# CESNET/GPUJPEG

Measured on AMD Instinct MI355X. Metric: Mpix/s encode+decode (8K RGB q75), higher is better.
Workload: dtype f32

## Files before the change

gpujpeg_amd/csrc/gj_dec_entropy_tok.hip:

```cpp
#include "gj_dec_internal.h"
#include "gj_bitreader.h"

#ifndef GJ_TOK_SUB
#define GJ_TOK_SUB 16
#define GJ_TOK_SUB_MAX 20
#endif
#define GJ_TOK_MAX_SUBS (GJ_TOK_CAP_U / GJ_TOK_SUB + (GJ_TOK_SUB <= 17 ? GJ_TOK_GMAX / 2 : GJ_TOK_GMAX))
#define GJ_TOK_WSTAGE 944
#define GJ_TOK_WG_PER_CU 4
#ifndef GJ_TOK_SYNC
#define GJ_TOK_SYNC 48
#endif
#define GJ_TOK_CHUNK_MAX 48

#ifdef GJ_TRACE_PHASES
static __device__ unsigned long long* gj_trace_buf;
extern "C" GJ_HIP_API int gj_hip_trace_set(void* p) { return hipMemcpyToSymbol(HIP_SYMBOL(gj_trace_buf), &p, sizeof p) == hipSuccess ? 0 : -1; }
#define GJ_TRACE(slot) do { if (threadIdx.x == 0 && gj_trace_buf) gj_trace_buf[(size_t)blockIdx.x * 16 + (slot)] = __builtin_amdgcn_s_memrealtime(); } while (0)
#else
#define GJ_TRACE(slot) ((void)0)
#endif

#ifdef GJ_TOK_STATS
extern "C" GJ_HIP_API unsigned long long gj_tok_stats[64];
unsigned long long gj_tok_stats[64];
#define GJ_STAT_WAVE(sm, i, lane, sym) do { gj_wave_sync(); (sm).statsym[threadIdx.x] = (sym); gj_wave_sync(); if ((lane) == 0) { \
    unsigned long long s_ = 0, m_ = 0; for (int q_ = 0; q_ < 64; q_++) { const unsigned v_ = (sm).statsym[(threadIdx.x & ~63) + q_]; s_ += v_; if (v_ > m_) m_ = v_; } \
    GJ_STAT(i, s_); GJ_STAT((i) + 1, 64 * m_); GJ_STAT((i) + 2, 1); } } while (0)
#define GJ_SYMS(c) (((c) >> 16) + 2u * ((c) & 0xFFFFu))
#define GJ_STAT(i, n) __atomic_fetch_add(&gj_tok_stats[i], (unsigned long long)(n), __ATOMIC_RELAXED)
#else
#define GJ_STAT(i, n) ((void)0)
#define GJ_STAT_WAVE(sm, i, lane, sym) ((void)0)
#endif

#ifndef GJ_TOK_WIN
#define GJ_TOK_WIN 1
#endif
#if GJ_TOK_WIN == 1
#define GJ_TOK_WIN_INIT(sm, p1) uint32_t wcur_ = (p1) >> 5, w0_ = (sm).U[wcur_], w1_ = (sm).U[wcur_ + 1], wnx_ = 0
#define GJ_TOK_WIN_BITS(sm, p1) wnx_ = (sm).U[wcur_ + 2]; const uint32_t win = __builtin_amdgcn_alignbit(w0_, w1_, ~(p1))
#define GJ_TOK_WIN_STEP(p1) do { const uint32_t wn_ = (p1) >> 5; const bool cross_ = wn_ != wcur_; w0_ = cross_ ? w1_ : w0_; w1_ = cross_ ? wnx_ : w1_; wcur_ = wn_; } while (0)
#else
#define GJ_TOK_WIN_INIT(sm, p1) ((void)0)
#define GJ_TOK_WIN_BITS(sm, p1) const uint32_t wi = (p1) >> 5; const uint32_t win = __builtin_amdgcn_alignbit((sm).U[wi], (sm).U[wi + 1], ~(p1))
#define GJ_TOK_WIN_STEP(p1) ((void)0)
#endif


struct GjTokLds {
    uint32_t U[GJ_TOK_CAP_U / 4 + 8];
    __attribute__((aligned(16))) uint16_t tab[2 * GJ_DEC2_WORDS];
    __attribute__((aligned(8))) uint2 rec[GJ_TOK_MAX_SUBS];
    __attribute__((aligned(16))) uint16_t pool[(GJ_TOK_MAX_BLOCKS + GJ_TOK_GMAX) * 2 + 4 * GJ_TOK_WSTAGE];
    uint32_t bb[GJ_TOK_GMAX + 1], cap[GJ_TOK_GMAX + 1], first[GJ_TOK_GMAX];
    uint16_t tabsel[GJ_TOK_GMAX];
    uint32_t sbit[GJ_TOK_GMAX], ebit[GJ_TOK_GMAX], sub0[GJ_TOK_GMAX + 1];
    uint32_t tmp[4];
    uint32_t nwork[2], big;
    uint32_t gpos;
    uint8_t zz[64 + 64];
#ifdef GJ_TOK_STATS
    uint32_t statsym[256];
#endif
};

__device__ __forceinline__ uint32_t gj_tok_run_in(const GjTokLds& sm, const uint32_t from, const uint32_t start_bit)
{
    uint32_t p1 = from - 1u;
    const uint32_t e1 = start_bit - 1u;
    uint32_t z = 1;
    uint32_t toff = (uint32_t)GJ_DEC2_WORDS * 2u;
    GJ_TOK_WIN_INIT(sm, p1);
    while (p1 < e1) {
        GJ_TOK_WIN_BITS(sm, p1);
        const uint16_t* t = reinterpret_cast<const uint16_t*>(reinterpret_cast<const uint8_t*>(sm.tab) + toff);
        uint32_t e = t[gj_bfe_u32<32 - GJ_DEC_FAST_BITS, GJ_DEC_FAST_BITS>(win)];
        if ((e & 31u) == 0) e = t[(e >> 5) + ((win >> 16) & 63u)];
        p1 += e & 31u;
        GJ_TOK_WIN_STEP(p1);
        z += (e >> 9) & 63u;
        const uint32_t inside = (uint32_t)((int32_t)(z - 64u) >> 31);
        z &= inside;
        toff = ((uint32_t)GJ_DEC2_WORDS * 2u) & inside;
    }
    return (p1 - e1) | (z << 5);
}

template <int MODE>
__device__ __forceinline__ uint32_t gj_tok_decode(const GjTokLds& sm, const uint32_t start_bit, const uint32_t end_bit, const uint32_t entry, uint32_t& counts,
                                                  uint16_t* __restrict__ tok_out ,
                                                  uint32_t* __restrict__ s_blkinfo ,
                                                  const uint32_t tok_rel , uint32_t blk,
                                                  const uint32_t nblocks, int16_t* __restrict__ coefs ,
                                                  uint32_t* __restrict__ s_big)
{
    uint32_t p1 = start_bit + (entry & 31u) - 1u;
    const uint32_t e1 = end_bit - 1u;
    uint32_t z = (entry >> 5) & 63u;
    uint32_t toff = z == 0 ? 0u : (uint32_t)GJ_DEC2_WORDS * 2u;
    uint32_t nb = 0, ntok = 0, mx = 0;
    uint16_t* tp = tok_out;
    GJ_TOK_WIN_INIT(sm, p1);
    while (p1 < e1) {
        GJ_TOK_WIN_BITS(sm, p1);
        const uint16_t* t = reinterpret_cast<const uint16_t*>(reinterpret_cast<const uint8_t*>(sm.tab) + toff);
        uint32_t e = t[gj_bfe_u32<32 - GJ_DEC_FAST_BITS, GJ_DEC_FAST_BITS>(win)];
        if ((e & 31u) == 0) e = t[(e >> 5) + ((win >> 16) & 63u)];
        const uint32_t tot = e & 31u, adv = (e >> 9) & 63u, sz = (e >> 5) & 15u;
        if (MODE == 0) {
            ntok += e >> 15;
        } else {
            const uint32_t x = win << (tot - sz);
            uint32_t neg = (uint32_t)((int32_t)~x >> 31);
            GJ_KEEP(neg);
            const uint32_t mag = (x ^ neg) >> ((32u - sz) & 31u);
            const int v = (int)((mag ^ neg) - neg);
            if ((int16_t)e < 0) {
                const uint32_t pos = z + adv - 1u;
                if (MODE == 1) {
                    mx = max(mx, sz);
                    *tp++ = (uint16_t)(((uint32_t)v << 6) | sm.zz[pos]);
                } else {
                    if (blk + nb < nblocks && pos < 64u) coefs[(uint64_t)(blk + nb) * 64 + sm.zz[pos]] = (int16_t)v;
                    ntok++;
                }
            } else if (z == 0) {
                const uint32_t t = MODE == 1 ? tok_rel + (uint32_t)(tp - tok_out) : tok_rel + ntok;
                if (blk + nb <= nblocks) s_blkinfo[blk + nb] = (sz ? (uint32_t)v & 0xFFFFu : 0u) | (t << 16);
            }
        }
        p1 += tot;
        GJ_TOK_WIN_STEP(p1);
        z += adv;
        const uint32_t inside = (uint32_t)((int32_t)(z - 64u) >> 31);
        z &= inside;
        toff = ((uint32_t)GJ_DEC2_WORDS * 2u) & inside;
        nb += 1u + inside;
    }
    if (MODE == 1) ntok = (uint32_t)(tp - tok_out);
    if (MODE == 1 && mx >= 10u) *s_big = 1u;
    counts = nb | (ntok << 16);
    return (p1 - e1) | (z << 5);
}

template <bool COOP>
__global__ __launch_bounds__(256, GJ_TOK_WG_PER_CU) void k_huffman_decode_tok(const gj_geom g, const uint8_t* __restrict__ jpeg, uint64_t jpeg_size,
                                                               const uint32_t* __restrict__ seg_pos, const uint32_t* __restrict__ seg_len,
                                                               const uint32_t* __restrict__ seg_index, const int seg_count_max,
                                                               const uint32_t* __restrict__ seg_count_ptr, const GjBatchPlan plan,
                                                               const uint16_t* __restrict__ tabs, int16_t* __restrict__ coefs,
                                                               uint16_t* __restrict__ d_tok, const uint32_t tok_cap, uint2* __restrict__ d_rec,
                                                               uint32_t* __restrict__ overflow, const GjFold F)
{
    constexpr int CAP_U = GJ_TOK_CAP_U, MAX_BLOCKS = GJ_TOK_MAX_BLOCKS, GMAX = GJ_TOK_GMAX, MAX_SUBS = GJ_TOK_MAX_SUBS;
    if (g.fb.sizes != nullptr) {
        const size_t z = blockIdx.z;
        jpeg += z * g.fb.jpeg;
        jpeg_size = g.fb.sizes[z];
        seg_pos += z * g.fb.seg; seg_len += z * g.fb.seg; seg_index += z * g.fb.seg;
        if (seg_count_ptr) seg_count_ptr += z * (sizeof(gj_scan_summary) / 4);
        overflow += z * (sizeof(gj_scan_summary) / 4);
        coefs += z * g.fb.coefs; d_tok += z * g.fb.tok; d_rec += z * g.fb.rec;
    }
    __shared__ GjTokLds sm;
    constexpr int POOL = sizeof(sm.pool) / 2;
    uint32_t* const s_stage = sm.U + 1;
    uint16_t* const s_pool = sm.pool;
    uint32_t* const s_blkinfo = reinterpret_cast<uint32_t*>(sm.pool);
    uint2* const s_rec = sm.rec;
    uint32_t *const s_bb = sm.bb, *const s_cap = sm.cap, *const s_first = sm.first, *const s_sbit = sm.sbit, *const s_ebit = sm.ebit, *const s_sub0 = sm.sub0;
    uint32_t* const s_tmp = sm.tmp;
    constexpr int BORROW = ((4 * GMAX + 1) * 2 + 7) & ~7;
    uint32_t* const s_pos = reinterpret_cast<uint32_t*>(s_pool + POOL - BORROW);
    uint32_t* const s_len = s_pos + GMAX;
    uint32_t* const s_ubyte = s_len + GMAX;
    uint32_t* const s_ulen = s_ubyte + GMAX + 1;
    static_assert(BORROW <= GJ_TOK_WSTAGE && MAX_SUBS <= POOL - BORROW, "borrowed space");
    uint16_t* const s_work = s_pool;

    const int tid = threadIdx.x, lane = tid & 63, wave = tid >> 6;
    GJ_TRACE(0);
    uint32_t sel_of_lane = 0x0C0C0C0Cu;
    {
        int at = 3;
#pragma unroll
        for (int k = 0; k < 4; k++)
            if (lane & (1 << k)) { sel_of_lane = (sel_of_lane & ~(0xFFu << (8 * at))) | ((uint32_t)k << (8 * at)); at--; }
    }
    if (tid < 128) sm.zz[tid] = tid < 64 ? GJ_ZZ[tid] : 0;
    if (tid == 0) sm.U[0] = 0;
    const uint32_t* end = reinterpret_cast<const uint32_t*>((reinterpret_cast<uintptr_t>(jpeg) + jpeg_size + 3) & ~(uintptr_t)3);

    int pc = 0;
    while (pc + 1 < plan.n && (int)blockIdx.x >= plan.batch0[pc + 1]) pc++;
    const int G = plan.g[pc];
    const int si0 = plan.first[pc] + ((int)blockIdx.x - plan.batch0[pc]) * G;
    uint32_t ld_s = 0xFFFFFFFFu, ld_p = 0, ld_l = 0;
    if (F.recs == nullptr && tid < G && si0 + tid < seg_count_max) { ld_s = seg_index[si0 + tid]; ld_p = seg_pos[si0 + tid]; ld_l = seg_len[si0 + tid]; }
    const int seg_count = seg_count_ptr ? min((int)*seg_count_ptr, seg_count_max) : seg_count_max;
    if (si0 >= seg_count) return;
    const int nseg = min(min(G, plan.first[pc] + plan.count[pc] - si0), seg_count - si0);
    if (F.recs != nullptr) {
        static_assert(GJ_FOLD_SCRATCH_WORDS(GJ_TOK_GMAX) * 2 <= (GJ_TOK_MAX_BLOCKS + GJ_TOK_GMAX) * 2, "fold scratch inside the block slots");
        if (!gj_fold_batch<GJ_TOK_GMAX>(F, g, jpeg, jpeg_size, plan, pc, si0, nseg, reinterpret_cast<uint32_t*>(sm.pool), s_tmp, ld_s, ld_p, ld_l)) return;
    }
    uint32_t loaded_tabs = 0xFFFFFFFFu;
    auto load_tables = [&](const uint32_t tb) {
        const uint4* src0 = reinterpret_cast<const uint4*>(tabs + (tb & 0xFFu) * GJ_DEC2_WORDS);
        const uint4* src1 = reinterpret_cast<const uint4*>(tabs + (tb >> 8) * GJ_DEC2_WORDS);
        uint4* dst = reinterpret_cast<uint4*>(sm.tab);
        for (int t = tid; t < GJ_DEC2_WORDS / 8; t += 256) { dst[t] = src0[t]; dst[GJ_DEC2_WORDS / 8 + t] = src1[t]; }
        loaded_tabs = tb;
    };
    if (plan.n > 1 && plan.n == g.comp_count) load_tables((uint32_t)(g.comp[pc].dc_table * 2 + 0) | ((uint32_t)(g.comp[pc].ac_table * 2 + 1) << 8));
    uint32_t my_pos = 0, my_len = 0, my_nblk = 0;
    {
        uint32_t first = 0, tb = 0;
        if (tid < nseg) {
            const uint32_t s = ld_s, p_ = ld_p, l_ = ld_l;
            if (s < (uint32_t)g.segment_count) {
                const GjSeg sg = gj_segment(g, (int)s);
                const gj_comp_geom& kc = g.comp[sg.comp];
                my_nblk = (uint32_t)sg.nblocks;
                my_pos = p_;
                my_len = l_;
                first = (uint32_t)(kc.data_offset / 64) + (uint32_t)sg.mcu_first;
                tb = (uint32_t)(kc.dc_table * 2 + 0) | ((uint32_t)(kc.ac_table * 2 + 1) << 8);
                if (((my_len + 3u) & ~3u) + 8u > (uint32_t)CAP_U || my_nblk > (uint32_t)MAX_BLOCKS) {
                    *overflow = 1u;
                    my_len = 0;
                    my_nblk = 0;
                }
            }
        }
        if (tid < GMAX) {
            s_first[tid] = first;
            sm.tabsel[tid] = (uint16_t)tb;
        }
        if (wave == 0) {
            s_bb[tid + 1] = gj_wave_incl_scan(tid < nseg ? my_nblk + 1u : 0u);
            s_cap[tid + 1] = gj_wave_incl_scan(my_len ? ((my_len + 3u) & ~3u) + 8u : 0u);
        }
        if (tid == 0) { s_bb[0] = 0; s_cap[0] = 0; sm.nwork[0] = 0; sm.nwork[1] = 0; }
    }
    static_assert(GMAX == 64, "one wave holds the batch's segment table");
    __syncthreads();
    const uint32_t stage0 = (2u * s_bb[nseg] + 7u) & ~7u, stage_cap = (((uint32_t)POOL - stage0) >> 2) & ~7u;
    uint16_t* const stage = s_pool + stage0 + (uint32_t)wave * stage_cap;

    for (int j0 = 0; j0 < nseg;) {
        if (tid == 0) sm.big = 0;
        if (tid < nseg) { s_pos[tid] = my_pos; s_len[tid] = my_len; }
        {
            const unsigned long long mb = __ballot(lane >= j0 && lane < nseg && my_nblk != 0u);
            if (wave == 0 && lane == (mb ? (int)__builtin_ctzll(mb) : j0)) sm.gpos = my_pos;
        }
        const uint32_t tb = sm.tabsel[j0];
        const bool other = lane > j0 && lane < nseg && s_bb[lane + 1] - s_bb[lane] != 1u && sm.tabsel[lane] != tb;
        const unsigned long long mo = __ballot(other);
        const int jstop = mo ? (int)__builtin_ctzll(mo) : nseg;
        const unsigned long long mf = __ballot(lane + 1 > j0 && lane + 1 <= jstop && s_cap[lane + 1] - s_cap[j0] <= (uint32_t)CAP_U);
        const int j1 = max(j0 + 1, mf ? 64 - (int)__builtin_clzll(mf) : 0);
        const int ng = j1 - j0;
        if (COOP) {
            const uint32_t n16 = min((s_cap[j1] - s_cap[j0] + 16u + 4u + 15u) >> 4, (uint32_t)(sizeof(sm.U) / 16));
            uint4* const z = reinterpret_cast<uint4*>(sm.U);
            for (uint32_t t = (uint32_t)tid; t < n16; t += 256u) z[t] = uint4{0u, 0u, 0u, 0u};
        }
        __syncthreads();
        GJ_TRACE(1);

        if (tb != loaded_tabs) load_tables(tb);

        bool coop = false;
        if (COOP) {
            bool irregular = false;
            if (lane < ng) {
                const int j = j0 + lane;
                irregular = s_len[j] == 0 || (lane + 1 < ng && s_pos[j + 1] != s_pos[j] + s_len[j] + 2u);
            }
            const uint32_t A = s_pos[j0], total = s_pos[j1 - 1] + s_len[j1 - 1] - A;
            coop = __ballot(irregular) == 0ull && total <= 256u * GJ_TOK_CHUNK_MAX && A >= 8u && (uint64_t)A + total <= jpeg_size;
        }
        if (coop) {
            const uint32_t A = s_pos[j0], total = s_pos[j1 - 1] + s_len[j1 - 1] - A;
            const uint32_t C = (((total + 255u) >> 8) + 3u) & ~3u;
            const uint32_t off0 = (uint32_t)tid * C;
            const uintptr_t a = reinterpret_cast<uintptr_t>(jpeg) + A + off0;
            const uint32_t* src = reinterpret_cast<const uint32_t*>(a & ~(uintptr_t)3) - 1;
            const uint32_t lead = (uint32_t)((reinterpret_cast<uintptr_t>(jpeg) + A) & 3);
            uint32_t win[GJ_TOK_CHUNK_MAX / 4 + 3];
#pragma unroll
            for (int i = 0; i < GJ_TOK_CHUNK_MAX / 4 + 3; i++) {
                win[i] = 0;
                if ((uint32_t)i < C / 4 + 3u && off0 < total + 4u && src + i < end) win[i] = src[i];
            }
            constexpr int ND = GJ_TOK_CHUNK_MAX / 4;
            uint64_t keep = 0, mark = 0;
            {
                const uint32_t K7 = 0x7F7F7F7Fu, K8 = 0x80808080u;
                uint32_t eq_prev = 0, m2_prev = 0, st_prev = 0;
                uint32_t ffc = 0;
                if (off0 != 0) {
                    const uint32_t x = __builtin_amdgcn_alignbyte(win[1], win[0], lead);
                    ffc = ((x & K7) + 0x01010101u) & x & K8;
                }
#pragma unroll
                for (int i = 0; i <= ND; i++) {
                    if ((uint32_t)(4 * i) <= C) {
                        const uint32_t x = __builtin_amdgcn_alignbyte(win[i + 2], win[i + 1], lead);
                        const uint32_t t = x & K7;
                        const uint32_t eq = (t + 0x01010101u) & x & K8;
                        const uint32_t zr = ~((t + K7) | x) & K8;
                        const uint32_t y = (x ^ 0xD0D0D0D0u) & 0xF8F8F8F8u;
                        const uint32_t rz = ~(((y & K7) + K7) | y) & K8;
                        const uint32_t before = __builtin_amdgcn_alignbit(eq, ffc, 24);
                        ffc = eq;
                        const uint32_t m2 = before & rz, st = before & zr;
                        if (i > 0) {
                            const uint32_t m1 = eq_prev & __builtin_amdgcn_alignbit(m2, m2_prev, 8);
                            const uint32_t kp = K8 & ~(st_prev | m2_prev | m1);
                            keep |= (uint64_t)((((kp >> 7) * 0x01020408u) >> 24) & 15u) << (4 * (i - 1));
                            mark |= (uint64_t)((((m1 >> 7) * 0x01020408u) >> 24) & 15u) << (4 * (i - 1));
                        }
                        eq_prev = eq; m2_prev = m2; st_prev = st;
                    }
                }
                const uint32_t nvalid = off0 >= total ? 0u : min(total - off0, C);
                const uint64_t valid = nvalid >= 64u ? ~0ull : (1ull << nvalid) - 1ull;
                keep &= valid;
                mark &= valid;
            }
            const uint32_t nkeep = (uint32_t)__popcll(keep), nmark = (uint32_t)__popcll(mark);
            uint32_t tot;
            const uint32_t inc = gj_wg256_incl_scan(nkeep | (nmark << 16), s_tmp, &tot);
            uint32_t o = (inc & 0xFFFFu) - nkeep, m = (inc >> 16) - nmark;
            coop = (tot >> 16) == (uint32_t)(ng - 1);
            if (coop) {
#pragma unroll
                for (int i = 0; i < ND; i++) {
                    if ((uint32_t)(4 * i) < C) {
                        const uint32_t x = __builtin_amdgcn_alignbyte(win[i + 2], win[i + 1], lead);
                        const uint32_t nk = (uint32_t)(keep >> (4 * i)) & 15u, nm = (uint32_t)(mark >> (4 * i)) & 15u;
                        const uint32_t below = nm ? ((nm & (0u - nm)) - 1u) : 15u;
                        const uint32_t nA = nk & below, nB = nk & ~below;
                        const uint32_t cA = (uint32_t)__popc(nA);
                        const uint32_t compA = __builtin_amdgcn_perm(0u, x, (uint32_t)__builtin_amdgcn_ds_bpermute((int)(nA << 2), (int)sel_of_lane));
                        const uint32_t compB = __builtin_amdgcn_perm(0u, x, (uint32_t)__builtin_amdgcn_ds_bpermute((int)(nB << 2), (int)sel_of_lane));
                        const uint32_t pA = o + 8u * m, pB = pA + cA + 8u;
                        const uint32_t shA = 8u * (pA & 3u), shB = 8u * (pB & 3u);
                        uint32_t* const dA = s_stage + (pA >> 2);
                        uint32_t* const dB = s_stage + (pB >> 2);
                        atomicOr(dA, compA >> shA);
                        atomicOr(dA + 1, __builtin_amdgcn_alignbit(compA, 0u, shA));
                        atomicOr(dB, compB >> shB);
                        atomicOr(dB + 1, __builtin_amdgcn_alignbit(compB, 0u, shB));
                        uint32_t mm = m;
                        for (uint32_t q = nm; q; q &= q - 1u) {
                            mm++;
                            s_ubyte[j0 + (int)mm] = o + (uint32_t)__popc(nk & ((q & (0u - q)) - 1u)) + 8u * mm;
                        }
                        m = mm;
                        o += (uint32_t)__popc(nk);
                    }
                }
                if (tid == 255) s_ubyte[j1] = o + 8u * m + 8u;
                if (tid == 0) s_ubyte[j0] = 0;
            }
        }
        __syncthreads();
        if (tid == 0) GJ_STAT(coop ? 30 : 31, 1);
        if (coop) {
            if (tid >= j0 && tid < j1) s_ulen[tid] = s_ubyte[tid + 1] - s_ubyte[tid] - 8u;
        } else {
            for (int j = j0 + wave; j < j1; j += 4) {
                const uint32_t len = s_len[j], base = s_cap[j] - s_cap[j0];
                uint32_t ulen = 0;
                if (len) {
                    const uintptr_t a = reinterpret_cast<uintptr_t>(jpeg) + s_pos[j];
                    const uint32_t* src = reinterpret_cast<const uint32_t*>(a & ~(uintptr_t)3);
                    const uint32_t ndw = ((uint32_t)(a & 3) + len + 3u) >> 2;
                    uint32_t w0 = 0;
                    if ((uint32_t)lane < ndw && src + lane < end) w0 = src[lane];
                    ulen = gj_unstuff_segment(jpeg, end, s_pos[j], len, s_stage, base, lane, w0);
                }
                if (lane == 0) { s_ubyte[j] = base; s_ulen[j] = ulen; }
            }
        }
        __syncthreads();

        GJ_TRACE(2);
        uint32_t sub_bytes = GJ_TOK_SUB;
        {
            uint32_t ulen = 0;
            if (tid >= j0 && tid < j1) {
                ulen = my_nblk ? s_ulen[tid] : 0u;
                s_sbit[tid] = s_ubyte[tid] * 8u + 32u;
                s_ebit[tid] = (s_ubyte[tid] + ulen) * 8u + 32u;
            }
            uint32_t tot;
            uint32_t a = gj_wg256_incl_scan(((ulen + GJ_TOK_SUB - 1) / GJ_TOK_SUB) | (ulen << 16), s_tmp, &tot) & 0xFFFFu;
            const uint32_t passes = ((tot & 0xFFFFu) + 255u) >> 8, bytes = tot >> 16;
            if (passes >= 2) {
#pragma unroll
                for (uint32_t s = GJ_TOK_SUB + 1; s <= GJ_TOK_SUB_MAX; s++)
                    if (sub_bytes == GJ_TOK_SUB && bytes / s + (uint32_t)ng <= 256u * (passes - 1u)) sub_bytes = s;
            }
            sub_bytes = (uint32_t)__builtin_amdgcn_readfirstlane((int)sub_bytes);
            if (sub_bytes != GJ_TOK_SUB) a = gj_wg256_incl_scan((ulen + sub_bytes - 1u) / sub_bytes, s_tmp, &tot);
            if (tid >= j0 && tid < j1) s_sub0[tid + 1] = min(a, (uint32_t)MAX_SUBS);
            if (tid == 0) s_sub0[j0] = 0;
        }
        __syncthreads();
        const int nsub = (int)s_sub0[j1];
        const uint32_t sub_bits = sub_bytes * 8u;
        if (tid == 0) { GJ_STAT(32 + min(nsub / 32, 31), 1); GJ_STAT(28, sub_bytes != GJ_TOK_SUB ? 1 : 0); }
        for (int k = tid; k < nsub; k += 256) {
            int lo = j0, hi = j1;
            while (hi - lo > 1) {
                const int mid = (lo + hi) >> 1;
                if (s_sub0[mid] <= (uint32_t)k) lo = mid; else hi = mid;
            }
            s_rec[k].x = (uint32_t)lo << 22;
        }
        __syncthreads();

        GJ_TRACE(3);
        for (int k0 = 0; k0 < nsub; k0 += 256) {
            const int k = k0 + tid;
            uint32_t c0 = 0;
            if (k < nsub) {
                const int j = (int)(s_rec[k].x >> 22);
                const uint32_t i = (uint32_t)k - s_sub0[j];
                const uint32_t sb = s_sbit[j] + i * sub_bits, eb = min(sb + sub_bits, s_ebit[j]);
                const uint32_t e0 = i == 0 ? 0u : gj_tok_run_in(sm, sb - (uint32_t)GJ_TOK_SYNC, sb);
                const uint32_t x0 = gj_tok_decode<0>(sm, sb, eb, e0, c0, nullptr, nullptr, 0, 0, 0, nullptr, nullptr);
                s_rec[k] = make_uint2(e0 | (x0 << 11) | ((uint32_t)j << 22), c0);
            }
            GJ_STAT_WAVE(sm, 16, lane, GJ_SYMS(c0));
        }
        GJ_TRACE(4);
        for (int round = 0;; round++) {
            __syncthreads();
            uint32_t* const cnt = &sm.nwork[round & 1];
            for (int k0 = 0; k0 < nsub; k0 += 256) {
                const int k = k0 + tid;
                bool cand = false;
                if (k < nsub) {
                    const uint32_t x = s_rec[k].x;
                    cand = (uint32_t)k != s_sub0[x >> 22] && ((s_rec[k - 1].x >> 11) & 0x7FFu) != (x & 0x7FFu);
                }
                const unsigned long long m = __ballot(cand);
                uint32_t base = 0;
                if (lane == 0 && m) base = atomicAdd(cnt, (uint32_t)__popcll(m));
                base = (uint32_t)__builtin_amdgcn_readfirstlane((int)base);
                if (cand) s_work[base + (uint32_t)__popcll(m & ((1ull << lane) - 1ull))] = (uint16_t)k;
            }
            __syncthreads();
            const int nwork = (int)*cnt;
            if (tid == 0) { GJ_STAT(0, round == 0 ? nsub : 0); GJ_STAT(1 + min(round, 13), nwork); GJ_STAT(15, nwork == 0 ? round : 0); }
            if (tid == 0) sm.nwork[(round + 1) & 1] = 0;
            if (nwork == 0) break;
            for (int w = tid; w < nwork; w += 256) {
                const int k = s_work[w];
                const int j = (int)(s_rec[k].x >> 22);
                const uint32_t i = (uint32_t)k - s_sub0[j];
                const uint32_t sb = s_sbit[j] + i * sub_bits, eb = min(sb + sub_bits, s_ebit[j]);
                const uint32_t e = (s_rec[k - 1].x >> 11) & 0x7FFu;
                uint32_t c;
                const uint32_t x = gj_tok_decode<0>(sm, sb, eb, e, c, nullptr, nullptr, 0, 0, 0, nullptr, nullptr);
                s_rec[k] = make_uint2(e | (x << 11) | ((uint32_t)j << 22), c);
            }
        }

        GJ_TRACE(5);
        {
            uint32_t carry = 0;
            for (int k0 = 0; k0 < nsub; k0 += 256) {
                const int k = k0 + tid;
                const uint32_t v = k < nsub ? s_rec[k].y : 0;
                uint32_t tot;
                const uint32_t inc = gj_wg256_incl_scan(v, s_tmp, &tot);
                __syncthreads();
                if (k < nsub) s_rec[k].y = carry + inc;
                carry += tot;
            }
        }
        for (uint32_t b = s_bb[j0] + (uint32_t)tid; b < s_bb[j1]; b += 256) s_blkinfo[b] = 0xFFFF0000u;
        __syncthreads();

        GJ_TRACE(6);
        const uint32_t T = nsub > 0 ? s_rec[nsub - 1].y >> 16 : 0u;
        uint32_t gbase = 4u * sm.gpos;
        if (sm.gpos > tok_cap / 4u || T > tok_cap - gbase) gbase = 0xFFFFFFFFu;
        if (gbase != 0xFFFFFFFFu) {
            const int ka = (int)(((uint32_t)nsub * (uint32_t)wave) >> 2), kb = (int)(((uint32_t)nsub * (uint32_t)(wave + 1)) >> 2);
            for (int k0 = ka; k0 < kb;) {
                const uint32_t P0 = k0 > 0 ? s_rec[k0 - 1].y >> 16 : 0u;
                const uint32_t a0 = (gbase + P0) & 7u;
                const int kk = k0 + lane;
                const bool fits = kk < kb && a0 + ((s_rec[min(kk, nsub - 1)].y >> 16) - P0) <= stage_cap;
                const unsigned long long fm = __ballot(fits);
                const int n = fm == ~0ull ? 64 : __builtin_ctzll(~fm);
                gj_wave_sync();
                uint32_t c = 0;
                if (lane < n) {
                    const int j = (int)(s_rec[kk].x >> 22);
                    const uint32_t kf = s_sub0[j];
                    const uint32_t i = (uint32_t)kk - kf;
                    const uint32_t before_k = kk > 0 ? s_rec[kk - 1].y : 0u, before_f = kf > 0 ? s_rec[kf - 1].y : 0u;
                    const uint32_t sb = s_sbit[j] + i * sub_bits, eb = min(sb + sub_bits, s_ebit[j]);
                    gj_tok_decode<1>(sm, sb, eb, s_rec[kk].x & 0x7FFu, c, stage + a0 + ((before_k >> 16) - P0), s_blkinfo + s_bb[j], before_k >> 16,
                                     (before_k & 0xFFFFu) - (before_f & 0xFFFFu), s_bb[j + 1] - s_bb[j] - 1u, nullptr, &sm.big);
                }
                gj_wave_sync();
                GJ_STAT_WAVE(sm, 20, lane, GJ_SYMS(c));
                const uint32_t cnt = (s_rec[k0 + n - 1].y >> 16) - P0;
                uint16_t* const dst = d_tok + (size_t)(gbase + P0 - a0);
                for (uint32_t p = (uint32_t)lane; p * 8u < a0 + cnt; p += 64) {
                    const uint32_t lo = p * 8u, hi = lo + 8u;
                    if (lo >= a0 && hi <= a0 + cnt) {
                        *reinterpret_cast<uint4*>(dst + lo) = *reinterpret_cast<const uint4*>(stage + lo);
                    } else {
                        for (uint32_t s = max(lo, a0); s < min(hi, a0 + cnt); s++) dst[s] = stage[s];
                    }
                }
                k0 += n;
                if (lane == 0) { GJ_STAT(24, 1); GJ_STAT(25, n); GJ_STAT(26, k0 >= kb ? (kb - ka + 63) / 64 : 0); GJ_STAT(27, k0 >= kb ? 1 : 0); }
            }
        }
        __syncthreads();

        GJ_TRACE(7);
        const bool planes = sm.big != 0 || gbase == 0xFFFFFFFFu;
        if (planes) {
            for (int j = j0 + wave; j < j1; j += 4) {
                const uint32_t chunks = (s_bb[j + 1] - s_bb[j] - 1u) * 8u;
                for (uint32_t c = (uint32_t)lane; c < chunks; c += 64)
                    reinterpret_cast<uint4*>(coefs + (uint64_t)(s_first[j] + (c >> 3)) * 64)[c & 7u] = make_uint4(0, 0, 0, 0);
            }
            __syncthreads();
            for (int k = tid; k < nsub; k += 256) {
                const int j = (int)(s_rec[k].x >> 22);
                const uint32_t kf = s_sub0[j];
                const uint32_t i = (uint32_t)k - kf;
                const uint32_t before_k = k > 0 ? s_rec[k - 1].y : 0u, before_f = kf > 0 ? s_rec[kf - 1].y : 0u;
                const uint32_t sb = s_sbit[j] + i * sub_bits, eb = min(sb + sub_bits, s_ebit[j]);
                uint32_t c;
                gj_tok_decode<2>(sm, sb, eb, s_rec[k].x & 0x7FFu, c, nullptr, s_blkinfo + s_bb[j], 0, (before_k & 0xFFFFu) - (before_f & 0xFFFFu),
                                 s_bb[j + 1] - s_bb[j] - 1u, coefs + (uint64_t)s_first[j] * 64, nullptr);
            }
            __syncthreads();
        }

        for (int j = j0 + wave; j < j1; j += 4) {
            const uint32_t bb = s_bb[j];
            const int nblk = (int)(s_bb[j + 1] - bb) - 1;
            const uint32_t k_end = s_sub0[j + 1];
            const uint32_t seg_end = k_end > s_sub0[j] ? s_rec[k_end - 1].y >> 16 : 0u;
            int carry = 0;
            for (int kb0 = 0; kb0 < nblk; kb0 += 64) {
                const int kb = kb0 + lane;
                const uint32_t info = kb < nblk ? s_blkinfo[bb + kb] : 0xFFFF0000u;
                const uint32_t inc = gj_wave_incl_scan((uint32_t)(int)(int16_t)(info & 0xFFFFu));
                const int dc = carry + (int)inc;
                carry += (int)(uint32_t)__builtin_amdgcn_readlane((int)inc, 63);
                if (kb < nblk) {
                    const uint32_t r = s_first[j] + (uint32_t)kb;
                    if (planes) {
                        coefs[(uint64_t)r * 64] = (int16_t)dc;
                        d_rec[r] = make_uint2(0u, 0xFFFF0000u);
                    } else {
                        const uint32_t t0 = info >> 16, nx = s_blkinfo[bb + kb + 1] >> 16;
                        const uint32_t t1 = nx != 0xFFFFu ? nx : seg_end;
                        const bool seen = t0 != 0xFFFFu;
                        const uint32_t cnt = seen && t1 >= t0 ? min(t1 - t0, 63u) : 0u;
                        d_rec[r] = make_uint2(seen ? gbase + t0 : 0u, (cnt << 16) | ((uint32_t)dc & 0xFFFFu));
                    }
                }
            }
        }
        __syncthreads();
        GJ_TRACE(8);
        j0 = j1;
    }
}

void gj_launch_huffman_tok(const gj_dec_job* job, hipStream_t st)
{
    const gj_geom& g = job->g;
    const unsigned frames = job->batch.count > 1 ? job->batch.count : 1u;
    const GjBatchPlan plan = gj_plan_batches(job, GJ_TOK_CAP_U, GJ_TOK_MAX_BLOCKS, GJ_TOK_GMAX, frames > 1 ? 0u : GJ_TOK_RESIDENT);
    auto kernel = job->tune.dec_tok_nocoop ? k_huffman_decode_tok<false> : k_huffman_decode_tok<true>;
    GjFold F = {nullptr, nullptr, 0, 0, 0, nullptr, nullptr};
    const bool fold = gj_tok_folds_table(job);
    if (fold) {
        const gj_scan_deferred& sc = job->scan;
        F = GjFold{sc.recs, sc.lists, sc.wgs, sc.part_bytes, sc.begin, sc.h_summary, sc.h_maxlen_parts};
        *sc.maxlen_part_count = (uint32_t)plan.batch0[plan.n];
    }
    hipLaunchKernelGGL(kernel, dim3((unsigned)plan.batch0[plan.n], 1, frames), dim3(256), 0, st, g, job->d_jpeg, job->jpeg_size, job->d_seg_pos, job->d_seg_len, job->d_seg_index,
                       job->seg_count, fold ? nullptr : job->d_seg_count, plan, job->d_huff_tab2, job->d_coefs, (uint16_t*)job->d_tok, job->tok_cap, (uint2*)job->d_blkrec,
                       job->d_overflow, F);
}

bool gj_tok_folds_table(const gj_dec_job* job)
{
    const gj_geom& g = job->g;
    if (!job->scan.valid || job->batch.count > 1 || g.fb.sizes != nullptr || g.interleaved || g.restart_interval <= 0 || job->seg_count != g.segment_count) return false;
    if (job->scan.wgs > 256u || job->scan.h_summary == nullptr || job->scan.h_maxlen_parts == nullptr || job->scan.maxlen_part_count == nullptr) return false;
    const GjBatchPlan plan = gj_plan_batches(job, GJ_TOK_CAP_U, GJ_TOK_MAX_BLOCKS, GJ_TOK_GMAX, GJ_TOK_RESIDENT);
    return plan.n == g.comp_count && (uint32_t)plan.batch0[plan.n] <= job->scan.maxlen_capacity;
}
```

Measured before the change: 170,800.

## Cut barriers in token decoder: wave scans, direct sub-record ownership, early sync exit

Replaces the workgroup-wide scans for sub-segment counts with single-wave scans, since the segment table fits in one wave. Each segment's lanes now write owning-segment ids into the sub-records directly, replacing the per-sub binary search and its barrier. The resync loop now exits once no sub-segment's end state changed, and its barrier moves to the end of each round. The DC prefix pass handles two segments per wave iteration to raise overlap. A trace-stop hook is added for debugging. The changes remove barriers and redundant passes at the cost of more complex loop logic and extra register use.

After: 172,200 (median of 6 runs). Within noise of the previous version (+0.8%).

```diff
diff --git a/gpujpeg_amd/csrc/gj_dec_entropy_tok.hip b/gpujpeg_amd/csrc/gj_dec_entropy_tok.hip
--- a/gpujpeg_amd/csrc/gj_dec_entropy_tok.hip
+++ b/gpujpeg_amd/csrc/gj_dec_entropy_tok.hip
@@ -15,8 +15,11 @@
 
 #ifdef GJ_TRACE_PHASES
 static __device__ unsigned long long* gj_trace_buf;
+static __device__ int gj_trace_stop_d = 1 << 30;
 extern "C" GJ_HIP_API int gj_hip_trace_set(void* p) { return hipMemcpyToSymbol(HIP_SYMBOL(gj_trace_buf), &p, sizeof p) == hipSuccess ? 0 : -1; }
-#define GJ_TRACE(slot) do { if (threadIdx.x == 0 && gj_trace_buf) gj_trace_buf[(size_t)blockIdx.x * 16 + (slot)] = __builtin_amdgcn_s_memrealtime(); } while (0)
+extern "C" GJ_HIP_API int gj_hip_trace_stop_decoder(int n) { return hipMemcpyToSymbol(HIP_SYMBOL(gj_trace_stop_d), &n, sizeof n) == hipSuccess ? 0 : -1; }
+#define GJ_TRACE(slot) do { if (threadIdx.x == 0 && gj_trace_buf) gj_trace_buf[(size_t)blockIdx.x * 16 + (slot)] = __builtin_amdgcn_s_memrealtime(); \
+                            if ((slot) >= 1 && (slot) >= gj_trace_stop_d) __builtin_amdgcn_endpgm(); } while (0)
 #else
 #define GJ_TRACE(slot) ((void)0)
 #endif
@@ -57,7 +60,7 @@
     uint16_t tabsel[GJ_TOK_GMAX];
     uint32_t sbit[GJ_TOK_GMAX], ebit[GJ_TOK_GMAX], sub0[GJ_TOK_GMAX + 1];
     uint32_t tmp[4];
-    uint32_t nwork[2], big;
+    uint32_t nwork[2], big, moved;
     uint32_t gpos;
     uint8_t zz[64 + 64];
 #ifdef GJ_TOK_STATS
@@ -250,7 +253,7 @@
     uint16_t* const stage = s_pool + stage0 + (uint32_t)wave * stage_cap;
 
     for (int j0 = 0; j0 < nseg;) {
-        if (tid == 0) sm.big = 0;
+        if (tid == 0) { sm.big = 0; sm.moved = 0; }
         if (tid < nseg) { s_pos[tid] = my_pos; s_len[tid] = my_len; }
         {
             const unsigned long long mb = __ballot(lane >= j0 && lane < nseg && my_nblk != 0u);
@@ -394,13 +397,18 @@
         uint32_t sub_bytes = GJ_TOK_SUB;
         {
             uint32_t ulen = 0;
-            if (tid >= j0 && tid < j1) {
-                ulen = my_nblk ? s_ulen[tid] : 0u;
-                s_sbit[tid] = s_ubyte[tid] * 8u + 32u;
-                s_ebit[tid] = (s_ubyte[tid] + ulen) * 8u + 32u;
-            }
-            uint32_t tot;
-            uint32_t a = gj_wg256_incl_scan(((ulen + GJ_TOK_SUB - 1) / GJ_TOK_SUB) | (ulen << 16), s_tmp, &tot) & 0xFFFFu;
+            const bool mine = lane >= j0 && lane < j1;
+            if (mine) {
+                ulen = s_bb[lane + 1] - s_bb[lane] != 1u ? s_ulen[lane] : 0u;
+                if (wave == 0) {
+                    s_sbit[lane] = s_ubyte[lane] * 8u + 32u;
+                    s_ebit[lane] = (s_ubyte[lane] + ulen) * 8u + 32u;
+                }
+            }
+            uint32_t n = (ulen + GJ_TOK_SUB - 1) / GJ_TOK_SUB;
+            const uint32_t inc = gj_wave_incl_scan(n | (ulen << 16));
+            const uint32_t tot = (uint32_t)__builtin_amdgcn_readlane((int)inc, 63);
+            uint32_t a = inc & 0xFFFFu;
             const uint32_t passes = ((tot & 0xFFFFu) + 255u) >> 8, bytes = tot >> 16;
             if (passes >= 2) {
 #pragma unroll
@@ -408,23 +416,21 @@
                     if (sub_bytes == GJ_TOK_SUB && bytes / s + (uint32_t)ng <= 256u * (passes - 1u)) sub_bytes = s;
             }
             sub_bytes = (uint32_t)__builtin_amdgcn_readfirstlane((int)sub_bytes);
-            if (sub_bytes != GJ_TOK_SUB) a = gj_wg256_incl_scan((ulen + sub_bytes - 1u) / sub_bytes, s_tmp, &tot);
-            if (tid >= j0 && tid < j1) s_sub0[tid + 1] = min(a, (uint32_t)MAX_SUBS);
+            if (sub_bytes != GJ_TOK_SUB) {
+                n = (ulen + sub_bytes - 1u) / sub_bytes;
+                a = gj_wave_incl_scan(n);
+            }
+            if (mine) {
+                const uint32_t kend = min(a, (uint32_t)MAX_SUBS);
+                if (wave == 0) s_sub0[lane + 1] = kend;
+                for (uint32_t k = min(a - n, (uint32_t)MAX_SUBS) + (uint32_t)wave; k < kend; k += 4u) s_rec[k].x = (uint32_t)lane << 22;
+            }
             if (tid == 0) s_sub0[j0] = 0;
         }
         __syncthreads();
         const int nsub = (int)s_sub0[j1];
         const uint32_t sub_bits = sub_bytes * 8u;
         if (tid == 0) { GJ_STAT(32 + min(nsub / 32, 31), 1); GJ_STAT(28, sub_bytes != GJ_TOK_SUB ? 1 : 0); }
-        for (int k = tid; k < nsub; k += 256) {
-            int lo = j0, hi = j1;
-            while (hi - lo > 1) {
-                const int mid = (lo + hi) >> 1;
-                if (s_sub0[mid] <= (uint32_t)k) lo = mid; else hi = mid;
-            }
-            s_rec[k].x = (uint32_t)lo << 22;
-        }
-        __syncthreads();
 
         GJ_TRACE(3);
         for (int k0 = 0; k0 < nsub; k0 += 256) {
@@ -441,8 +447,8 @@
             GJ_STAT_WAVE(sm, 16, lane, GJ_SYMS(c0));
         }
         GJ_TRACE(4);
+        __syncthreads();
         for (int round = 0;; round++) {
-            __syncthreads();
             uint32_t* const cnt = &sm.nwork[round & 1];
             for (int k0 = 0; k0 < nsub; k0 += 256) {
                 const int k = k0 + tid;
@@ -462,16 +468,22 @@
             if (tid == 0) { GJ_STAT(0, round == 0 ? nsub : 0); GJ_STAT(1 + min(round, 13), nwork); GJ_STAT(15, nwork == 0 ? round : 0); }
             if (tid == 0) sm.nwork[(round + 1) & 1] = 0;
             if (nwork == 0) break;
+            bool moved = false;
             for (int w = tid; w < nwork; w += 256) {
                 const int k = s_work[w];
-                const int j = (int)(s_rec[k].x >> 22);
+                const uint32_t old = s_rec[k].x;
+                const int j = (int)(old >> 22);
                 const uint32_t i = (uint32_t)k - s_sub0[j];
                 const uint32_t sb = s_sbit[j] + i * sub_bits, eb = min(sb + sub_bits, s_ebit[j]);
                 const uint32_t e = (s_rec[k - 1].x >> 11) & 0x7FFu;
                 uint32_t c;
                 const uint32_t x = gj_tok_decode<0>(sm, sb, eb, e, c, nullptr, nullptr, 0, 0, 0, nullptr, nullptr);
+                moved |= x != ((old >> 11) & 0x7FFu);
                 s_rec[k] = make_uint2(e | (x << 11) | ((uint32_t)j << 22), c);
             }
+            if (__ballot(moved) != 0ull && lane == 0) sm.moved = (uint32_t)round + 1u;
+            __syncthreads();
+            if (sm.moved != (uint32_t)round + 1u) break;
         }
 
         GJ_TRACE(5);
@@ -554,31 +566,40 @@
             __syncthreads();
         }
 
-        for (int j = j0 + wave; j < j1; j += 4) {
-            const uint32_t bb = s_bb[j];
-            const int nblk = (int)(s_bb[j + 1] - bb) - 1;
-            const uint32_t k_end = s_sub0[j + 1];
-            const uint32_t seg_end = k_end > s_sub0[j] ? s_rec[k_end - 1].y >> 16 : 0u;
-            int carry = 0;
-            for (int kb0 = 0; kb0 < nblk; kb0 += 64) {
+        for (int j = j0 + wave; j < j1; j += 8) {
+            const int jB = j + 4;
+            const bool two = jB < j1;
+            const uint32_t bbA = s_bb[j], bbB = two ? s_bb[jB] : 0u;
+            const int nblkA = (int)(s_bb[j + 1] - bbA) - 1, nblkB = two ? (int)(s_bb[jB + 1] - bbB) - 1 : 0;
+            const uint32_t keA = s_sub0[j + 1], keB = two ? s_sub0[jB + 1] : 0u;
+            const uint32_t seg_endA = keA > s_sub0[j] ? s_rec[keA - 1].y >> 16 : 0u;
+            const uint32_t seg_endB = two && keB > s_sub0[jB] ? s_rec[keB - 1].y >> 16 : 0u;
+            const uint32_t firstA = s_first[j], firstB = two ? s_first[jB] : 0u;
+            int carryA = 0, carryB = 0;
+            for (int kb0 = 0; kb0 < max(nblkA, nblkB); kb0 += 64) {
                 const int kb = kb0 + lane;
-                const uint32_t info = kb < nblk ? s_blkinfo[bb + kb] : 0xFFFF0000u;
-                const uint32_t inc = gj_wave_incl_scan((uint32_t)(int)(int16_t)(info & 0xFFFFu));
-                const int dc = carry + (int)inc;
-                carry += (int)(uint32_t)__builtin_amdgcn_readlane((int)inc, 63);
-                if (kb < nblk) {
-                    const uint32_t r = s_first[j] + (uint32_t)kb;
+                const bool inA = kb < nblkA, inB = kb < nblkB;
+                const uint32_t infoA = inA ? s_blkinfo[bbA + kb] : 0xFFFF0000u, infoB = inB ? s_blkinfo[bbB + kb] : 0xFFFF0000u;
+                const uint32_t nxA = inA ? s_blkinfo[bbA + kb + 1] >> 16 : 0xFFFFu, nxB = inB ? s_blkinfo[bbB + kb + 1] >> 16 : 0xFFFFu;
+                const uint32_t incA = gj_wave_incl_scan((uint32_t)(int)(int16_t)(infoA & 0xFFFFu));
+                const uint32_t incB = gj_wave_incl_scan((uint32_t)(int)(int16_t)(infoB & 0xFFFFu));
+                const int dcA = carryA + (int)incA, dcB = carryB + (int)incB;
+                carryA += (int)(uint32_t)__builtin_amdgcn_readlane((int)incA, 63);
+                carryB += (int)(uint32_t)__builtin_amdgcn_readlane((int)incB, 63);
+                auto put = [&](const uint32_t r, const uint32_t info, const uint32_t nx, const uint32_t seg_end, const int dc) {
                     if (planes) {
                         coefs[(uint64_t)r * 64] = (int16_t)dc;
                         d_rec[r] = make_uint2(0u, 0xFFFF0000u);
                     } else {
-                        const uint32_t t0 = info >> 16, nx = s_blkinfo[bb + kb + 1] >> 16;
+                        const uint32_t t0 = info >> 16;
                         const uint32_t t1 = nx != 0xFFFFu ? nx : seg_end;
                         const bool seen = t0 != 0xFFFFu;
                         const uint32_t cnt = seen && t1 >= t0 ? min(t1 - t0, 63u) : 0u;
                         d_rec[r] = make_uint2(seen ? gbase + t0 : 0u, (cnt << 16) | ((uint32_t)dc & 0xFFFFu));
                     }
-                }
+                };
+                if (inA) put(firstA + (uint32_t)kb, infoA, nxA, seg_endA, dcA);
+                if (inB) put(firstB + (uint32_t)kb, infoB, nxB, seg_endB, dcB);
             }
         }
         __syncthreads();
```
